# mat-lee/tetris-reinforcement-learning

Hardware: NVIDIA B200
Metric: placements/sec (movegen) (higher is better)
Workload: dtype u16

## Files before the change

### __graft_entry__.py

```python
import os
import sys

ROOT = os.path.dirname(os.path.abspath(__file__))
if ROOT not in sys.path:
    sys.path.insert(0, ROOT)


def build():
    from tetris_reinforcement_learning_b200 import build as b
    so = b.build(force=b.needs_build())
    from oracle import oracle
    oracle.build()
    import tetris_reinforcement_learning_b200
    from tetris_reinforcement_learning_b200 import _native
    _native.lib()
    print("built", so)


def smoke():
    import numpy as np
    import torch
    assert torch.cuda.is_available(), "smoke() needs a CUDA device"
    from oracle import oracle
    from tetris_reinforcement_learning_b200 import env, move_generation, synth
    from tetris_reinforcement_learning_b200.state import games_equal

    boards, cur, alt = synth.movegen_workload(64, seed=1, caves=True)
    dev = torch.device("cuda:0")
    d_mask = torch.empty((boards.shape[0], 362), dtype=torch.int32, device=dev)
    d_n = torch.empty(boards.shape[0], dtype=torch.int16, device=dev)
    move_generation.movegen_device(torch.from_numpy(boards.view(np.int16)).to(dev),
                                   torch.from_numpy(cur).to(dev), torch.from_numpy(alt).to(dev),
                                   d_mask, None, d_n, None)
    torch.cuda.synchronize()
    want_masks, want_n, _, total = oracle.movegen_batch(boards, cur, alt)
    assert np.array_equal(d_mask.cpu().numpy().view(np.uint32), want_masks), "movegen mask mismatch"
    assert np.array_equal(d_n.cpu().numpy().view(np.uint16), want_n)
    from tetris_reinforcement_learning_b200 import _native
    _native.lib().trl_movegen_warp_form(2)
    try:
        d_mask.zero_()
        move_generation.movegen_device(torch.from_numpy(boards.view(np.int16)).to(dev), torch.from_numpy(cur).to(dev),
                                       torch.from_numpy(alt).to(dev), d_mask, None, d_n, None)
        torch.cuda.synchronize()
    finally:
        _native.lib().trl_movegen_warp_form(-1)
    assert np.array_equal(d_mask.cpu().numpy().view(np.uint32), want_masks), "movegen mask mismatch (two-pass form)"
    assert np.array_equal(d_n.cpu().numpy().view(np.uint16), want_n)

    seed = 3
    games = env.game_setup_host(128, 0, seed)
    shadow = oracle.game_setup(128, 0, seed)
    for _ in range(8):
        pl = games["players"][np.arange(128), games["turn"]]
        res = move_generation.movegen_host(np.ascontiguousarray(pl["rows"]), pl["piece"].copy(),
                                           np.where(pl["held"] != 255, pl["held"], pl["queue"][:, 0]).astype(np.uint8),
                                           want_mask=False, want_moves=True, moves_cap=128)
        moves = res["moves"][:, 0].astype(np.uint16)
        env.env_step_host(games, moves, True, seed)
        oracle.env_step(shadow, moves, True, seed)
    assert games_equal(games, shadow).all(), "env step mismatch"

    from tetris_reinforcement_learning_b200 import architectures as arch, trunk
    from tetris_reinforcement_learning_b200.config import Config
    from tetris_reinforcement_learning_b200.selfplay import SelfPlayEngine
    torch.manual_seed(0)
    mc = arch.AlphaSameConfig(blocks=10, filters=16)
    net = arch.AlphaSame(mc).to(dev).eval()
    grids = (torch.rand((30, 1, 40, 10), device=dev) < 0.3).float()
    with torch.no_grad():
        ref = net.grid_features(grids)
    got = trunk.trunk_forward(trunk.pack_alphasame_trunk(net), grids.to(torch.bfloat16)).float()
    err = (got - ref).abs().max().item()
    assert err <= 0.03 * ref.abs().max().item() + 0.02, f"trunk mismatch {err}"
    cfg = Config(visual=False, ruleset="s2", model="pytorch", model_config=mc, MAX_ITER=8, training=True)
    eng = SelfPlayEngine(cfg, trunk.make_fused_evaluator(net), 64, device=dev, seed=1, feature_dtype=torch.bfloat16, max_rounds=4)
    eng.step(120)
    samples, ends = eng.drain()
    assert len(samples) > 0 and (eng.get_ctl()["status"] == 0).all(), "self-play step failed"
    from tetris_reinforcement_learning_b200 import trunk_wide
    wnet = arch.AuxBaseResNet(arch.AuxBaseResNetConfig(blocks=2, filters=32)).to(dev).eval()
    wt = trunk_wide.WideTrunk(trunk_wide.pack_wide_trunk(wnet), dev)
    with torch.no_grad():
        wref = wnet.opp_collapse(wnet._process_grid(grids)).flatten(1)
    wgot = trunk_wide.wide_trunk_forward(wt, grids.to(torch.bfloat16)).float()[:, 4 * 400:]
    wt.check()
    werr = (wgot - wref).abs().max().item()
    assert werr <= 0.04 * wref.abs().max().item() + 0.03, f"wide trunk mismatch {werr}"
    print(f"smoke ok: {boards.shape[0]} movegen calls ({total} placements) and 8 plies x 128 games bit-exact vs oracle; "
          f"trunk max err {err:.4f}, wide trunk max err {werr:.4f}; {len(samples)} searches, {len(ends)} games finished")


if __name__ == "__main__":
    build()
    if len(sys.argv) > 1 and sys.argv[1] == "smoke":
        smoke()
```

### tetris_reinforcement_learning_b200/csrc/movegen_warp.cu

```cuda
#include <cuda_runtime.h>
#include <stdint.h>

#include <mutex>

#include "trl_common.cuh"
#include "trl_tables.cuh"

namespace {

constexpr int kFifoCap = 768;
__constant__ int c_fifo_limit = kFifoCap;
constexpr int kCallsPerBlock = 8;
constexpr int kWarps = 2 * kCallsPerBlock;
constexpr int kVRows = TRL_MAP_H + 2;

struct PieceState {
    uint32_t vv[4][kVRows];
    uint32_t fu[4][kVRows];
    union {
        uint16_t fifo[kFifoCap];
        struct {
            uint32_t tsnap[4][32];
            uint32_t tp[4][2][36];
        };
// ... 333 lines not shown
        }
        const uint32_t b_nhi = e0w0[R] & 0xFFFFu, b_u = e0w0[R] >> 16, b_nlo = e0w1[R] & 0xFFFFu;
        const uint32_t b_any = b_nhi | b_u | b_nlo, b_win = b_u & ~b_nhi;
        all_n |= b_nhi | b_nlo; all_u |= b_u;
        const uint32_t l_n = late[R] & 0xFFFFu, l_u = late[R] >> 16, has_late = l_n | l_u;
        const uint32_t early_win = (q_any & q_win) | (~q_any & ((b_any & b_win) | (~b_any & i_win)));
        const uint32_t win = (early & early_win) | (~early & a_win);
        const uint32_t qn = (early & q_n) | (~early & a_n), qu = (early & q_u) | (~early & a_u);
        const uint32_t dec_u = (has_late & l_u & ~l_n & ~qn) | (~has_late & win);
        const uint32_t decided = (has_late & ((l_u & ~l_n & ~qn) | (l_n & ~l_u & ~qu))) | ~has_late;
        const uint32_t mixed = all_n & all_u & placed;
        const uint32_t suspect = seed_cell | (b_any & ~early);
        if (mixed & ~(decided & ~suspect)) undecided = true;
#ifdef TRL_MOVEGEN_STATS
        if (__any_sync(kAll, mixed & ~early)) TRL_REASON(11);
        if (__any_sync(kAll, mixed & suspect)) TRL_REASON(12);
        if (__any_sync(kAll, mixed & ~suspect & ~decided)) TRL_REASON(13);
#endif
        ulk[R] = ((all_u & ~mixed) | (dec_u & mixed)) & 0xFFFFu;
    }
    if (__any_sync(kAll, undecided)) { TRL_REASON(14); return false; }
    TRL_REASON(15);
    ulkA = ulk[0] | (ulk[2] << 16);
    ulkB = ulk[1] | (ulk[3] << 16);
    return true;
}

constexpr uint32_t kMinos[7][4] = {
    {TRL_PK(0, 0, 1, 0, 1, 1, 2, 1), TRL_PK(1, 1, 1, 2, 2, 0, 2, 1), TRL_PK(0, 1, 1, 1, 1, 2, 2, 2), TRL_PK(0, 1, 0, 2, 1, 0, 1, 1)},
    {TRL_PK(0, 1, 1, 1, 2, 0, 2, 1), TRL_PK(1, 0, 1, 1, 1, 2, 2, 2), TRL_PK(0, 1, 0, 2, 1, 1, 2, 1), TRL_PK(0, 0, 1, 0, 1, 1, 1, 2)},
    {TRL_PK(0, 0, 0, 1, 1, 0, 1, 1), TRL_PK(0, 0, 0, 1, 1, 0, 1, 1), TRL_PK(0, 0, 0, 1, 1, 0, 1, 1), TRL_PK(0, 0, 0, 1, 1, 0, 1, 1)},
    {TRL_PK(0, 1, 1, 0, 1, 1, 2, 0), TRL_PK(1, 0, 1, 1, 2, 1, 2, 2), TRL_PK(0, 2, 1, 1, 1, 2, 2, 1), TRL_PK(0, 0, 0, 1, 1, 1, 1, 2)},
    {TRL_PK(0, 1, 1, 1, 2, 1, 3, 1), TRL_PK(2, 0, 2, 1, 2, 2, 2, 3), TRL_PK(0, 2, 1, 2, 2, 2, 3, 2), TRL_PK(1, 0, 1, 1, 1, 2, 1, 3)},
    {TRL_PK(0, 0, 0, 1, 1, 1, 2, 1), TRL_PK(1, 0, 1, 1, 1, 2, 2, 0), TRL_PK(0, 1, 1, 1, 2, 1, 2, 2), TRL_PK(0, 2, 1, 0, 1, 1, 1, 2)},
    {TRL_PK(0, 1, 1, 0, 1, 1, 2, 1), TRL_PK(1, 0, 1, 1, 1, 2, 2, 1), TRL_PK(0, 1, 1, 1, 1, 2, 2, 1), TRL_PK(0, 1, 1, 0, 1, 1, 1, 2)},
};

template <int TYPE, int R>
__device__ __forceinline__ uint32_t validity_row(const uint32_t (&e)[4]) {
    constexpr uint32_t mm = kMinos[TYPE][R];
    constexpr int c0 = mm & 15, r0 = (mm >> 4) & 15, c1 = (mm >> 8) & 15, r1 = (mm >> 12) & 15;
    constexpr int c2 = (mm >> 16) & 15, r2 = (mm >> 20) & 15, c3 = (mm >> 24) & 15, r3 = (mm >> 28) & 15;
    return 0x3FFFu & (e[r0] >> c0) & (e[r1] >> c1) & (e[r2] >> c2) & (e[r3] >> c3);
}

template <int TYPE>
__device__ __forceinline__ void validity_rows(const uint32_t (&e)[4], uint32_t (&v)[4]) {
    v[0] = validity_row<TYPE, 0>(e);
    v[1] = validity_row<TYPE, 1>(e);
    v[2] = validity_row<TYPE, 2>(e);
    v[3] = validity_row<TYPE, 3>(e);
}

template <bool SPECIAL, class St>
__device__ __forceinline__ bool search_piece_rows(St& S, const uint16_t* rows, int hi, int type, bool via_hold, uint32_t* mask) {
    const int lane = threadIdx.x & 31;
    const int sx = trl_spawn_x(type);
    const bool is_T = (type == P_T);
    const int my = lane + kWin0;
    uint32_t e[4];
#pragma unroll
    for (int k = 0; k < 4; ++k) e[k] = trl_empty_row(rows, my - 2 + k) << 2;
    uint32_t VA = 0u, VB = 0u;
    if (SPECIAL && TRL_ROWS_SPECIAL_V) {
        uint32_t v[4];
        switch (type) {
            case 0: validity_rows<0>(e, v); break;
            case 1: validity_rows<1>(e, v); break;
            case 2: validity_rows<2>(e, v); break;
            case 3: validity_rows<3>(e, v); break;
            case 4: validity_rows<4>(e, v); break;
            case 5: validity_rows<5>(e, v); break;
            default: validity_rows<6>(e, v); break;
        }
        VA = v[0] | (v[2] << 16);
        VB = v[1] | (v[3] << 16);
    } else {
#pragma unroll 1
    for (int r = 0; r < 4; ++r) {
        const uint32_t m4 = c_minos[type][r];
        uint32_t acc = 0x3FFFu;
#pragma unroll
        for (int m = 0; m < 4; ++m) {
            const uint32_t co = (m4 >> (8 * m)) & 15u, ro = (m4 >> (8 * m + 4)) & 15u;
            const uint32_t ek = ro == 0 ? e[0] : (ro == 1 ? e[1] : (ro == 2 ? e[2] : e[3]));
            acc &= ek >> co;
        }
        const uint32_t sh = acc << (16 * (r >> 1));
        if (r & 1) VB |= sh; else VA |= sh;
    }
    }
    {
        const int pad = lane < 2 ? lane : lane + 32;
        S.vv[0][lane + 2] = VA << 2;
        S.vv[1][lane + 2] = VB << 2;
        if (lane < 4) { S.vv[0][pad] = 0u; S.vv[1][pad] = 0u; }
#pragma unroll
        for (int r = 0; r < 4; ++r) {
            S.fu[r][lane + 2] = 0u;
            if (lane < 4) S.fu[r][pad] = 0u;
        }
    }
    const uint32_t v_spawn = __shfl_sync(0xffffffffu, VA, TRL_SPAWN_Y + 2 - kWin0);
    if (via_hold && !((v_spawn >> (sx + 2)) & 1u)) return true;
    const int slane = max(hi - (int)c_matrix_size[type], TRL_SPAWN_Y) + 2 - kWin0;
    const uint32_t vs = __shfl_sync(0xffffffffu, VA, slane);
    if (!((vs >> (sx + 2)) & 1u)) return true;
// ... 91 lines not shown
                        __syncwarp();
                        const uint32_t d = S.fu[nrot][lane + 2];
                        const uint32_t k0 = (((nrot & 1) ? a0B : a0A) >> (16 * (nrot >> 1))) & 0xFFFFu;
                        if (round < 8) tt[((round * 4 + nrot) * 3 + kd) * 32 + lane] |= d | k0;
                        S.fu[nrot][lane + 2] = saved | d;
                        a0A |= sA; a0B |= sB;
                        __syncwarp();
                    }
                } trace_end{S, ttrace, nrot, kd, lane, tround, t_saved, t_a0A, t_a0B, a0A, a0B};
#endif
                const uint32_t Vn = ((nrot & 1) ? VB : VA) >> (16 * (nrot >> 1));
                const uint32_t c0 = ne & Vn;
                const uint32_t c0s = c0 << (16 * (nrot >> 1));
                if (nrot & 1) a0B |= c0s; else a0A |= c0s;
                uint32_t rem = ne & ~c0;
                if (!__any_sync(0xffffffffu, rem)) continue;
                const TrlKicks& K = c_kicks[tab][r][kd];
                const int kn = K.n;
                const uint32_t* vt = &S.vv[nrot & 1][lane + 2];
                const int vsh = 2 + 16 * (nrot >> 1);
                uint32_t* at = &S.fu[nrot][lane + 2];
#pragma unroll 1
                for (int ki = 1; ki < kn; ++ki) {
                    TRL_STAT(5);
                    const int kx = K.k[ki][0], ky = K.k[ki][1];
                    const uint32_t cand = rem & (vt[-ky] >> (kx + vsh));
                    rem &= ~cand;
                    if (cand) {
                        uint32_t arr = (cand << 4) >> (4 - kx);
                        if (is_T && kd != 1 && ki == kn - 1) arr <<= 16;
                        atomicOr(&at[-ky], arr);
                    }
                    if (!__any_sync(0xffffffffu, rem)) break;
                }
            }
        }
        }
#ifdef TRL_T_TRACE
        ++tround;
#endif
        __syncwarp();
        {
            const uint32_t f0 = S.fu[0][lane + 2], f1 = S.fu[1][lane + 2], f2 = S.fu[2][lane + 2], f3 = S.fu[3][lane + 2];
#ifdef TRL_MOVEGEN_STATS
            if (is_T && stat_2 == 1) {
                const uint32_t stA = VA & ~dA, stB = VB & ~dB;
                const uint32_t mA = (((f0 | a0A) & (f0 >> 16)) & 0xFFFFu) | ((((f2 << 16) | a0A) & f2) & 0xFFFF0000u);
                const uint32_t mB = (((f1 | a0B) & (f1 >> 16)) & 0xFFFFu) | ((((f3 << 16) | a0B) & f3) & 0xFFFF0000u);
                if (__any_sync(0xffffffffu, (mA & stA) | (mB & stB))) stat_6 = 1;
            }
#endif
            RA |= a0A | ((f0 | (f0 >> 16)) & 0xFFFFu) | ((f2 | (f2 >> 16)) << 16);
            RB |= a0B | ((f1 | (f1 >> 16)) & 0xFFFFu) | ((f3 | (f3 >> 16)) << 16);
            if (is_T && ++kick_rounds == 2) {
                S.tsnap[0][lane] = f0 | (a0A & 0xFFFFu); S.tsnap[1][lane] = f1 | (a0B & 0xFFFFu);
                S.tsnap[2][lane] = f2 | (a0A >> 16); S.tsnap[3][lane] = f3 | (a0B >> 16);
                S.fu[0][lane + 2] = 0u; S.fu[1][lane + 2] = 0u; S.fu[2][lane + 2] = 0u; S.fu[3][lane + 2] = 0u;
                a0A = 0u; a0B = 0u;
                snapped = true;
                __syncwarp();
            }
        }
    }
#ifdef TRL_MOVEGEN_STATS
    if (lane == 0) {
        atomicAdd(&g_fast_stats[2], (unsigned long long)stat_2); atomicAdd(&g_fast_stats[3], (unsigned long long)stat_3);
        atomicAdd(&g_fast_stats[4], (unsigned long long)stat_4); atomicAdd(&g_fast_stats[5], (unsigned long long)stat_5);
        atomicAdd(&g_fast_stats[6], (unsigned long long)stat_6);
    }
#endif
    if (__any_sync(0xffffffffu, lane < 2 && (RA | RB))) return false;
    const uint32_t placedA = RA & ~dA, placedB = RB & ~dB;
#ifdef TRL_T_TRACE
    if (ttrace) {
        ttrace[8 * 4 * 3 * 32 + 0 * 32 + lane] = placedA & 0xFFFFu; ttrace[8 * 4 * 3 * 32 + 1 * 32 + lane] = placedB & 0xFFFFu;
        ttrace[8 * 4 * 3 * 32 + 2 * 32 + lane] = placedA >> 16; ttrace[8 * 4 * 3 * 32 + 3 * 32 + lane] = placedB >> 16;
        ttrace[8 * 4 * 3 * 32 + 4 * 32 + lane] = (uint32_t)rows[lane] | (lane < TRL_ROWS - 32 ? (uint32_t)rows[lane + 32] << 16 : 0u);
    }
#endif
    uint32_t flagA = 0u, flagB = 0u, ulkA = 0u, ulkB = 0u;
    if (is_T) {
        uint32_t nA = a0A, nB = a0B, uA = 0u, uB = 0u;
#pragma unroll
        for (int r = 0; r < 4; ++r) {
            const uint32_t fw = S.fu[r][lane + 2] | (snapped ? S.tsnap[r][lane] : 0u);
            const uint32_t n = (fw & 0xFFFFu) << (16 * (r >> 1)), u = (fw >> 16) << (16 * (r >> 1));
            if (r & 1) { nB |= n; uB |= u; } else { nA |= n; uA |= u; }
        }
        flagA = nA | uA; flagB = nB | uB;
        ulkA = uA; ulkB = uB;
        const uint32_t mxA = nA & uA & placedA, mxB = nB & uB & placedB;
        const uint32_t mixed_rots = (__any_sync(0xffffffffu, mxA & 0xFFFFu) ? 1u : 0u) | (__any_sync(0xffffffffu, mxB & 0xFFFFu) ? 2u : 0u) |
                                    (__any_sync(0xffffffffu, mxA >> 16) ? 4u : 0u) | (__any_sync(0xffffffffu, mxB >> 16) ? 8u : 0u);
        if (mixed_rots) {
            if (!t_order_decide(S, lane, VA, VB, slane, sx + 2, placedA, placedB, a0A, a0B, snapped, mixed_rots, ulkA, ulkB)) return false;
        }
    }
    const int pbase = c_plane_base[type];
    const int nrot_planes = c_plane_nrot[type];
    const bool zsi = (type == P_Z || type == P_S || type == P_I);
    if (my < TRL_MAP_H - 1) {
        const int n_rot = (type == P_O) ? 1 : 4;
#pragma unroll 1
        for (int rot = 0; rot < n_rot; ++rot) {
            const uint32_t placed = (((rot & 1) ? placedB : placedA) >> (16 * (rot >> 1))) & 0xFFFFu;
            if (!placed) continue;
            int row = my - 2;
            uint32_t bits = placed;
            if (zsi) {
                if (rot == 2) row += 1;
                else if (rot == 3) bits >>= 1;
            }
            if (!is_T) {
                or_chunk(mask, pbase + rot % nrot_planes, row, bits & 0x7FFu);
            } else {
                const uint32_t f = (((rot & 1) ? flagB : flagA) >> (16 * (rot >> 1))) & placed;
                const uint32_t u = (((rot & 1) ? ulkB : ulkA) >> (16 * (rot >> 1))) & 0xFFFFu;
                or_chunk(mask, pbase + rot, row, (placed & ~f) & 0x7FFu);
                or_chunk(mask, pbase + 4 + rot, row, (f & ~u) & 0x7FFu);
                or_chunk(mask, pbase + 8 + rot, row, (f & u) & 0x7FFu);
            }
        }
    }
    return true;
}

__device__ __noinline__ bool search_piece_rows_call(PieceState& S, const uint16_t* rows, int type, bool via_hold, uint32_t* mask) {
    return search_piece_rows<false>(S, rows, first_block_row(rows, threadIdx.x & 31), type, via_hold, mask);
}

__device__ __noinline__ void search_piece_fifo(PieceState& S, const uint16_t* rows, int type, bool via_hold, uint32_t* mask,
                                  uint32_t& status, const uint32_t (*kpack)[4][3][2]) {
    const int lane = threadIdx.x & 31;
    uint32_t minos[4];
#pragma unroll
    for (int r = 0; r < 4; ++r) minos[r] = c_minos[type][r];
    const int sx = trl_spawn_x(type);
    if (via_hold && !trl_fits(rows, minos[0], sx, TRL_SPAWN_Y)) return;

#pragma unroll
    for (int r = 0; r < 4; ++r) {
        for (int my = lane; my < kVRows; my += 32) {
            S.vv[r][my] = (my < TRL_MAP_H) ? trl_valid_row(rows, minos[r], my) : 0u;
            S.fu[r][my] = 0u;
        }
    }
    int hi = TRL_ROWS;
    for (int i = lane; i < TRL_ROWS; i += 32)
        if (rows[i] & TRL_FULL_ROW) hi = min(hi, i);
    hi = __reduce_min_sync(0xffffffffu, hi);
    const int sy = max(hi - (int)c_matrix_size[type], TRL_SPAWN_Y);
    __syncwarp();
    if (!((S.vv[0][sy + 2] >> (sx + 2)) & 1u)) return;

    const bool is_T = (type == P_T);
    const bool rotates = (type != P_O);
    const int tab = (type == P_I) ? 1 : 0;

    uint32_t head = 0, tail = 1;
    if (lane == 0) S.fifo[0] = (uint16_t)fifo_pack(sx + 2, sy + 2, 0, 0, 0);
    __syncwarp();

    while (head != tail) {
        const int n = min(32u, tail - head);
        const uint32_t e = (lane < n) ? S.fifo[(head + lane) % kFifoCap] : 0u;
        const int mx = e & 15, my = (e >> 4) & 63, rot = (e >> 10) & 3;
        const uint32_t bit = 1u << mx;
        const uint32_t w = S.vv[rot][my];
        const bool stuck = !(S.vv[rot][my + 1] & bit);
        const bool need = (lane < n) && !((w >> 16) & bit) && (w & bit);
        const uint32_t m_need = __ballot_sync(0xffffffffu, need);
        const int first = m_need ? (__ffs(m_need) - 1) : 32;
        if (is_T) {
            const bool emit = (lane < n) && (lane <= first) && ((e >> 12) & 1u) && stuck;
            const uint32_t m_emit = __ballot_sync(0xffffffffu, emit);
            if (m_emit) {
                const bool u = (e >> 13) & 1u;
                const uint32_t m_true = __ballot_sync(0xffffffffu, emit && u);
                if (m_true == 0u || m_true == m_emit) {
                    if (emit) flag_cell(&S.fu[rot][my], bit, u);
                } else if (emit) {
                    const uint32_t grp = __match_any_sync(m_emit, e & 0xFFFu);
                    if ((31 - __clz(grp)) == lane) flag_cell(&S.fu[rot][my], bit, u);
                    else atomicOr(&S.fu[rot][my], bit);
                }
// ... 180 lines not shown
                        if (mixed && lane != l) { __syncwarp(); continue; }
                        uint32_t iv = Im[0] | Im[1] | Im[2];
                        while (iv) {
                            const int ex = __ffs(iv) - 1;
                            iv &= iv - 1;
#pragma unroll
                            for (int kd = 0; kd < 3; ++kd) {
                                if (!((Im[kd] >> ex) & 1u)) continue;
                                const int ki = ((k0[kd] >> ex) & 1u) | (((k1[kd] >> ex) & 1u) << 1) | (((k2[kd] >> ex) & 1u) << 2);
                                const int kn = c_kicks[tab][frot][kd].n;
                                const bool nulk = (kd != 1 && ki == kn - 1);
                                const int kx = (int)(((*kpack)[frot][kd][0] >> (4 * ki)) & 15u) - 2;
                                const int ky = (int)(((*kpack)[frot][kd][1] >> (4 * ki)) & 15u) - 2;
                                flag_cell(&S.fu[(frot + kd + 1) & 3][ky_row - ky], 1u << (ex + kx), nulk);
                            }
                        }
                        __syncwarp();
                    }
                }
            }
            __syncwarp();
        }
    }
    __syncwarp();

    const int pbase = c_plane_base[type];
    const int nrot_planes = c_plane_nrot[type];
    const bool zsi = (type == P_Z || type == P_S || type == P_I);
    for (int rot = 0; rot < 4; ++rot) {
        if (type == P_O && rot > 0) break;
        for (int my = 2 + lane; my < TRL_MAP_H - 1; my += 32) {
            const uint32_t wv = S.vv[rot][my];
            const uint32_t placed = (wv >> 16) & ~S.vv[rot][my + 1] & 0xFFFFu;
            if (!placed) continue;
            int row = my - 2;
            uint32_t bits = placed;
            if (zsi) {
                if (rot == 2) row += 1;
                else if (rot == 3) bits >>= 1;
            }
            if (!is_T) {
                or_chunk(mask, pbase + rot % nrot_planes, row, bits & 0x7FFu);
            } else {
                const uint32_t fw = S.fu[rot][my];
                const uint32_t f = fw & placed, u = fw >> 16;
                or_chunk(mask, pbase + rot, row, (placed & ~f) & 0x7FFu);
                or_chunk(mask, pbase + 4 + rot, row, (f & ~u) & 0x7FFu);
                or_chunk(mask, pbase + 8 + rot, row, (f & u) & 0x7FFu);
            }
        }
    }
}

__device__ __forceinline__ void search_piece_warp(PieceState& S, const uint16_t* rows, int type, bool via_hold, uint32_t* mask,
                                                  uint32_t& status, const uint32_t (*kpack)[4][3][2], bool exact_only = false) {
    if (!exact_only && c_fast_path && c_fifo_limit == kFifoCap) {
        const bool done = search_piece_rows_call(S, rows, type, via_hold, mask);
        if ((threadIdx.x & 31) == 0) atomicAdd(&g_fast_stats[done ? 0 : 1], 1ull);
        if (done) return;
        __syncwarp();
    }
    search_piece_fifo(S, rows, type, via_hold, mask, status, kpack);
}

__device__ __noinline__ void write_move_list(const CallState& C, int lane, uint16_t* mv, int cap) {
    uint32_t nz = 0u;
#pragma unroll
    for (int j = 0; j < 12; ++j) {
        const int w = lane + 32 * j;
        if (w < TRL_MASK_WORDS && C.mask[w]) nz |= 1u << j;
    }
    while (nz) {
        const int j = __ffs(nz) - 1;
        nz &= nz - 1;
        const int w = lane + 32 * j;
        uint32_t m = C.mask[w];
        int pos = (int)C.lbase[(w * 683) >> 13] + (int)C.woff[w];
        while (m) {
            const int b = __ffs(m) - 1;
            m &= m - 1;
            if (pos < cap) mv[pos] = (uint16_t)(w * 32 + b);
            ++pos;
        }
    }
}

template <int MODE = 0>
__device__ __forceinline__ void write_call_outputs(CallState& C, int i, int lane, uint32_t* __restrict__ mask_bits,
                                                   uint16_t* __restrict__ moves, int moves_cap,
                                                   uint16_t* __restrict__ n_moves, uint32_t* __restrict__ status,
                                                   uint16_t* __restrict__ compact, unsigned long long compact_cap,
                                                   unsigned long long* __restrict__ compact_total,
                                                   unsigned long long* __restrict__ offsets) {
    if (C.skip) {
        if (lane == 0) {
            if (n_moves) n_moves[i] = 0;
            if (status) status[i] = 0;
            if (compact) offsets[i] = 0;
        }
        return;
    }
    const int w0 = lane * 12;
    const bool want_list = MODE == 0 ? (compact != nullptr || moves != nullptr) : (MODE == 2);
    int cnt = 0;
    uint32_t* gm = mask_bits ? mask_bits + (size_t)i * TRL_MASK_WORDS : nullptr;
#pragma unroll 1
// ... 148 lines not shown
    __shared__ uint32_t s_kpack[2][4][3][2];
    const int tid = threadIdx.x, warp = tid >> 5, lane = tid & 31;
    SoloState& S = reinterpret_cast<SoloState*>(smem_raw)[warp];
    CallState& C = S.C;
    if (tid < 24) {
        const int t = tid / 12, r = (tid / 3) % 4, kd = tid % 3;
        const TrlKicks& K = c_kicks[t][r][kd];
        uint32_t px = 0, py = 0;
        for (int ki = 0; ki < K.n; ++ki) {
            px |= (uint32_t)(K.k[ki][0] + 2) << (4 * ki);
            py |= (uint32_t)(K.k[ki][1] + 2) << (4 * ki);
        }
        s_kpack[t][r][kd][0] = px;
        s_kpack[t][r][kd][1] = py;
    }
    __syncthreads();
    const int n_items = call_list ? (int)call_count[0] : n;
#pragma unroll 1
    for (int j = blockIdx.x * kSoloWarps + warp; j < n_items; j += gridDim.x * kSoloWarps) {
        const int i = call_list ? call_list[j] : j;
        int c, a, skip;
        zero_mask(C, lane);
        stage_call(C, i, lane, boards, cur, alt, games, index, c, a, skip);
        __syncwarp();
        if (!skip) {
            uint32_t st = 0;
#pragma unroll 1
            for (int which = 0; which < 2; ++which) {
                const int type = which ? a : c;
                if (type == TRL_NONE || (which && a == c)) continue;
                search_piece_warp(S.P, C.rows, type, which != 0, C.mask, st, &s_kpack[type == P_I ? 1 : 0],
                                  call_list != nullptr && type == P_T);
                __syncwarp();
            }
            st = __reduce_or_sync(0xffffffffu, st);
            if (st && lane == 0) C.status |= st;
            __syncwarp();
        }
        write_call_outputs(C, i, lane, mask_bits, moves, moves_cap, n_moves, status, compact, compact_cap, compact_total, offsets);
        __syncwarp();
    }
}

#ifndef TRL_ROWS_SPECIAL
#define TRL_ROWS_SPECIAL 1
#endif
#ifndef TRL_ROWS_WARPS
#define TRL_ROWS_WARPS 4
#endif
#ifndef TRL_ROWS_MIN_BLOCKS
#define TRL_ROWS_MIN_BLOCKS 10
#endif
constexpr int kRowsWarps = TRL_ROWS_WARPS;

struct RowsState {
    uint32_t vv[2][kWinRows];
    uint32_t fu[4][kWinRows];
    uint32_t tsnap[4][32];
    uint32_t tp[4][2][36];
};

struct RowsWarp {
    RowsState P;
    CallState C;
};

template <bool WANT_LIST>
__global__ void __launch_bounds__(kRowsWarps * 32, TRL_ROWS_MIN_BLOCKS)
movegen_rows_kernel(const uint16_t* __restrict__ boards, const uint8_t* __restrict__ cur,
                    const uint8_t* __restrict__ alt, const TrlGame* __restrict__ games,
                    const int32_t* __restrict__ index, int n, uint32_t* __restrict__ mask_bits,
                    uint16_t* __restrict__ moves, int moves_cap, uint16_t* __restrict__ n_moves,
                    uint32_t* __restrict__ status, uint16_t* __restrict__ compact, unsigned long long compact_cap,
                    unsigned long long* __restrict__ compact_total, unsigned long long* __restrict__ offsets,
                    int32_t* __restrict__ undecided, uint32_t* __restrict__ undecided_count) {
    extern __shared__ __align__(16) uint8_t smem_raw[];
    const int tid = threadIdx.x, warp = tid >> 5, lane = tid & 31;
    RowsWarp& S = reinterpret_cast<RowsWarp*>(smem_raw)[warp];
    CallState& C = S.C;
    const int i = blockIdx.x * kRowsWarps + warp;
    if (i >= n) return;
    int c, a, skip;
    zero_mask(C, lane);
    stage_call(C, i, lane, boards, cur, alt, games, index, c, a, skip);
    __syncwarp();
    if (!skip) {
        const int hi = first_block_row(C.rows, lane);
        bool ok = true;
#pragma unroll 1
        for (int which = 0; which < 2 && ok; ++which) {
            const int type = which ? a : c;
            if (type == TRL_NONE || (which && a == c)) continue;
            ok = search_piece_rows<TRL_ROWS_SPECIAL != 0>(S.P, C.rows, hi, type, which != 0, C.mask);
            if (ok) TRL_REASON(0); else TRL_REASON(1);
            __syncwarp();
        }
        if (!ok) {
            if (lane == 0) undecided[atomicAdd(undecided_count, 1u)] = i;
            return;
        }
    }
    write_call_outputs<WANT_LIST ? 2 : 1>(C, i, lane, mask_bits, moves, moves_cap, n_moves, status, compact, compact_cap, compact_total, offsets);
}

constexpr int kListSlots = 16;

__device__ __forceinline__ void slot_barrier(int slot) {
    asm volatile("bar.sync %0, 64;" ::"r"(slot) : "memory");
}

__global__ void __launch_bounds__(kListSlots * 64)
movegen_list_kernel(const TrlGame* __restrict__ games, const int32_t* __restrict__ index,
                    const int32_t* __restrict__ list, uint32_t* __restrict__ count_done,
                    uint16_t* __restrict__ moves, int moves_cap, uint16_t* __restrict__ n_moves, int rounds,
                    TrlSearchCtl* __restrict__ ctl) {
    extern __shared__ __align__(16) uint8_t smem_raw[];
    PieceState* ps = reinterpret_cast<PieceState*>(smem_raw);
    CallState* cs = reinterpret_cast<CallState*>(smem_raw + sizeof(PieceState) * kListSlots * 2);
    __shared__ int s_ticket[kListSlots];
    __shared__ uint32_t s_kpack[2][4][3][2];
    const int tid = threadIdx.x, warp = tid >> 5, lane = tid & 31;
    const int slot = warp >> 1, which = warp & 1;
    __shared__ int s_count;
    __shared__ unsigned s_warps_done;
    if (tid == 32) { s_count = (int)count_done[0]; s_warps_done = 0u; }
    {
        if (tid < 24) {
            const int t = tid / 12, r = (tid / 3) % 4, kd = tid % 3;
            const TrlKicks& K = c_kicks[t][r][kd];
            uint32_t px = 0, py = 0;
            for (int ki = 0; ki < K.n; ++ki) {
                px |= (uint32_t)(K.k[ki][0] + 2) << (4 * ki);
                py |= (uint32_t)(K.k[ki][1] + 2) << (4 * ki);
            }
            s_kpack[t][r][kd][0] = px;
            s_kpack[t][r][kd][1] = py;
        }
    }
    __syncthreads();
    const int count = s_count;
    const int n_work = min((int)gridDim.x, (count + kListSlots * rounds - 1) / (kListSlots * rounds));
    if ((int)blockIdx.x < n_work) {
        CallState& C = cs[slot];
        while (true) {
            if (which == 0 && lane == 0) s_ticket[slot] = (int)atomicAdd(&count_done[2], 1u);
            slot_barrier(slot);
            const int j = s_ticket[slot];
            if (j >= count) break;
            const int g = list[j];
            const int gi = index[g];
            for (int w2 = which * 32 + lane; w2 < TRL_MASK_WORDS + 2; w2 += 64) C.mask[w2] = 0u;
            if (which == 0) {
                const TrlPlayer& p = games[gi].players[games[gi].turn & 1];
                for (int r = lane; r < TRL_ROWS; r += 32) C.rows[r] = p.rows[r];
                int c = p.piece;
// ... 79 lines not shown
    if (!rc) rc = trl_check(cudaMemcpyToSymbol(g_fast_stats, z, sizeof(z)));
    answered[0] = h[0]; answered[1] = h[1];
#ifdef TRL_MOVEGEN_STATS
    for (int k = 2; k < 16; ++k) answered[k] = h[k];
#endif
    return rc;
}

extern "C" int trl_debug_movegen_t_trace(uint32_t* device_buffer, unsigned cap) {
#ifdef TRL_T_TRACE
    unsigned zero = 0;
    int rc = trl_check(cudaMemcpyToSymbol(g_t_trace, &device_buffer, sizeof(device_buffer)));
    if (!rc) rc = trl_check(cudaMemcpyToSymbol(g_t_trace_cap, &cap, sizeof(cap)));
    if (!rc) rc = trl_check(cudaMemcpyToSymbol(g_t_trace_n, &zero, sizeof(zero)));
    return rc ? rc : kTTraceWords;
#else
    (void)device_buffer; (void)cap;
    return TRL_E_ARG;
#endif
}

extern "C" int trl_debug_movegen_fifo_limit(int limit) {
    if (limit < 1 || limit > kFifoCap) limit = kFifoCap;
    g_fifo_limit_host = limit;
    return trl_check(cudaMemcpyToSymbol(c_fifo_limit, &limit, sizeof(int)));
}

int trl_launch_movegen_listed(const TrlGame* games, const int32_t* index, const int32_t* list, uint32_t* count_done,
                              uint16_t* moves, int moves_cap, uint16_t* n_moves, TrlSearchCtl* ctl, cudaStream_t stream) {
    if (!games || !index || !list || !count_done || !moves || !n_moves || moves_cap <= 0) return TRL_E_ARG;
    const size_t smem = sizeof(PieceState) * kListSlots * 2 + sizeof(CallState) * kListSlots;
    static int n_sm = 0;
    if (!n_sm) {
        int dev = 0, sms = 0;
        int rc = trl_check(cudaGetDevice(&dev));
        if (!rc) rc = trl_check(cudaDeviceGetAttribute(&sms, cudaDevAttrMultiProcessorCount, dev));
        if (!rc) rc = trl_check(cudaFuncSetAttribute(movegen_list_kernel, cudaFuncAttributeMaxDynamicSharedMemorySize, (int)smem));
        if (rc) return rc;
        n_sm = sms;
    }
    movegen_list_kernel<<<n_sm, kListSlots * 64, smem, stream>>>(games, index, list, count_done, moves, moves_cap, n_moves,
                                                                g_list_rounds, ctl);
    return trl_check(cudaGetLastError());
}

static int g_form = -1;
extern "C" void trl_movegen_warp_form(int form) { g_form = form; }

struct TwoPassScratch { cudaStream_t stream; uint32_t* buf; size_t cap; bool used; };
static TwoPassScratch g_scratch[8];

static std::mutex g_scratch_mutex;

static uint32_t* two_pass_scratch(cudaStream_t stream, int n) {
    std::lock_guard<std::mutex> lock(g_scratch_mutex);
    TwoPassScratch* slot = nullptr;
    for (auto& e : g_scratch) if (e.used && e.stream == stream) { slot = &e; break; }
    if (!slot) for (auto& e : g_scratch) if (!e.used) { slot = &e; e.used = true; e.stream = stream; e.buf = nullptr; e.cap = 0; break; }
    if (!slot) return nullptr;
    const size_t need = (size_t)n + 16;
    if (slot->cap < need) {
        cudaStreamCaptureStatus cs = cudaStreamCaptureStatusNone;
        if (cudaStreamIsCapturing(stream, &cs) != cudaSuccess || cs != cudaStreamCaptureStatusNone) return nullptr;
        if (slot->buf) { cudaStreamSynchronize(stream); cudaFree(slot->buf); slot->buf = nullptr; slot->cap = 0; }
        if (cudaMalloc(&slot->buf, need * sizeof(uint32_t)) != cudaSuccess) { cudaGetLastError(); return nullptr; }
        slot->cap = need;
    }
    return slot->buf;
}

int trl_launch_movegen_warp(const uint16_t* boards, const uint8_t* cur, const uint8_t* alt, const TrlGame* games,
                            const int32_t* index, int n, uint32_t* mask_bits, uint16_t* moves, int moves_cap,
                            uint16_t* n_moves, uint32_t* status, cudaStream_t stream, uint16_t* compact,
                            unsigned long long compact_cap, unsigned long long* compact_total,
                            unsigned long long* offsets) {
    static int n_sm = 0;
    static bool configured = false;
    const size_t smem_warp = sizeof(PieceState) * kWarps + sizeof(CallState) * kCallsPerBlock;
    const size_t smem_solo = sizeof(SoloState) * kSoloWarps;
    const size_t smem_rows = sizeof(RowsWarp) * kRowsWarps;
    if (!configured) {
        int dev = 0;
        int rc = trl_check(cudaGetDevice(&dev));
        if (!rc) rc = trl_check(cudaDeviceGetAttribute(&n_sm, cudaDevAttrMultiProcessorCount, dev));
        if (!rc) rc = trl_check(cudaFuncSetAttribute(movegen_warp_kernel, cudaFuncAttributeMaxDynamicSharedMemorySize, (int)smem_warp));
        if (!rc) rc = trl_check(cudaFuncSetAttribute(movegen_solo_kernel, cudaFuncAttributeMaxDynamicSharedMemorySize, (int)smem_solo));
        if (!rc) rc = trl_check(cudaFuncSetAttribute(movegen_solo_kernel, cudaFuncAttributePreferredSharedMemoryCarveout, 100));
        if (!rc) rc = trl_check(cudaFuncSetAttribute(movegen_rows_kernel<false>, cudaFuncAttributeMaxDynamicSharedMemorySize, (int)smem_rows));
        if (!rc) rc = trl_check(cudaFuncSetAttribute(movegen_rows_kernel<false>, cudaFuncAttributePreferredSharedMemoryCarveout, 100));
        if (!rc) rc = trl_check(cudaFuncSetAttribute(movegen_rows_kernel<true>, cudaFuncAttributeMaxDynamicSharedMemorySize, (int)smem_rows));
        if (!rc) rc = trl_check(cudaFuncSetAttribute(movegen_rows_kernel<true>, cudaFuncAttributePreferredSharedMemoryCarveout, 100));
        if (rc) return rc;
        configured = true;
    }
    int form = g_form < 0 ? (n >= 3 * 4736 ? 2 : 0) : g_form;
    if (form == 2 && (!g_fast_path_host || g_fifo_limit_host != kFifoCap)) form = 1;
    uint32_t* scratch = form == 2 ? two_pass_scratch(stream, n) : nullptr;
    if (form == 2 && !scratch) form = 1;
    if (form == 2) {
        int rc = trl_check(cudaMemsetAsync(scratch, 0, sizeof(uint32_t), stream));
        if (rc) return rc;
        if (moves || compact)
            movegen_rows_kernel<true><<<(n + kRowsWarps - 1) / kRowsWarps, kRowsWarps * 32, smem_rows, stream>>>(
                boards, cur, alt, games, index, n, mask_bits, moves, moves_cap, n_moves, status, compact, compact_cap,
                compact_total, offsets, (int32_t*)(scratch + 16), scratch);
        else
            movegen_rows_kernel<false><<<(n + kRowsWarps - 1) / kRowsWarps, kRowsWarps * 32, smem_rows, stream>>>(
                boards, cur, alt, games, index, n, mask_bits, moves, moves_cap, n_moves, status, compact, compact_cap,
                compact_total, offsets, (int32_t*)(scratch + 16), scratch);
        rc = trl_check(cudaGetLastError());
        if (rc) return rc;
        const int blocks = min(8 * n_sm, (n + kSoloWarps - 1) / kSoloWarps);
        movegen_solo_kernel<<<blocks, kSoloWarps * 32, smem_solo, stream>>>(
            boards, cur, alt, games, index, n, mask_bits, moves, moves_cap, n_moves, status, compact, compact_cap,
            compact_total, offsets, (const int32_t*)(scratch + 16), scratch);
        return trl_check(cudaGetLastError());
    }
    if (form == 1) {
        const int blocks = (n + kSoloWarps - 1) / kSoloWarps;
        movegen_solo_kernel<<<blocks, kSoloWarps * 32, smem_solo, stream>>>(boards, cur, alt, games, index, n, mask_bits, moves,
                                                                           moves_cap, n_moves, status, compact, compact_cap,
                                                                           compact_total, offsets, nullptr, nullptr);
        int rc = trl_check(cudaGetLastError());
        return rc;
    }
    const int blocks = (n + kCallsPerBlock - 1) / kCallsPerBlock;
    movegen_warp_kernel<<<blocks, kWarps * 32, smem_warp, stream>>>(boards, cur, alt, games, index, n, mask_bits, moves,
                                                                   moves_cap, n_moves, status, compact, compact_cap,
                                                                   compact_total, offsets, nullptr, nullptr);
    return trl_check(cudaGetLastError());
}
```

Baseline: 10.50 billion.

## Split T-piece order resolution into deferred passes instead of full fallback

The rows kernel no longer runs T-spin order resolution inline. Calls whose only failure is the T piece get their partial mask saved and are deferred to a new persistent T-order kernel, and calls it still cannot decide go to an exact FIFO kernel. Only other failures fall back to the legacy solo kernel. The aim is to shrink the rows kernel's shared-memory footprint (tsnap/tp removed) and to stop sending T-heavy calls down the expensive full re-search. In exchange it adds two extra launches, atomic work queues, and partial-mask storage traffic.

```diff
diff --git a/__graft_entry__.py b/__graft_entry__.py
--- a/__graft_entry__.py
+++ b/__graft_entry__.py
@@ -45,7 +45,7 @@
         torch.cuda.synchronize()
     finally:
         _native.lib().trl_movegen_warp_form(-1)
-    assert np.array_equal(d_mask.cpu().numpy().view(np.uint32), want_masks), "movegen mask mismatch (two-pass form)"
+    assert np.array_equal(d_mask.cpu().numpy().view(np.uint32), want_masks), "movegen mask mismatch (pass form)"
     assert np.array_equal(d_n.cpu().numpy().view(np.uint16), want_n)
 
     seed = 3
diff --git a/tetris_reinforcement_learning_b200/csrc/movegen_warp.cu b/tetris_reinforcement_learning_b200/csrc/movegen_warp.cu
--- a/tetris_reinforcement_learning_b200/csrc/movegen_warp.cu
+++ b/tetris_reinforcement_learning_b200/csrc/movegen_warp.cu
@@ -409,7 +409,7 @@
     v[3] = validity_row<TYPE, 3>(e);
 }
 
-template <bool SPECIAL, class St>
+template <bool SPECIAL, bool T_ORDER, class St>
 __device__ __forceinline__ bool search_piece_rows(St& S, const uint16_t* rows, int hi, int type, bool via_hold, uint32_t* mask) {
     const int lane = threadIdx.x & 31;
     const int sx = trl_spawn_x(type);
@@ -607,13 +607,15 @@
 #endif
             RA |= a0A | ((f0 | (f0 >> 16)) & 0xFFFFu) | ((f2 | (f2 >> 16)) << 16);
             RB |= a0B | ((f1 | (f1 >> 16)) & 0xFFFFu) | ((f3 | (f3 >> 16)) << 16);
-            if (is_T && ++kick_rounds == 2) {
-                S.tsnap[0][lane] = f0 | (a0A & 0xFFFFu); S.tsnap[1][lane] = f1 | (a0B & 0xFFFFu);
-                S.tsnap[2][lane] = f2 | (a0A >> 16); S.tsnap[3][lane] = f3 | (a0B >> 16);
-                S.fu[0][lane + 2] = 0u; S.fu[1][lane + 2] = 0u; S.fu[2][lane + 2] = 0u; S.fu[3][lane + 2] = 0u;
-                a0A = 0u; a0B = 0u;
-                snapped = true;
-                __syncwarp();
+            if constexpr (T_ORDER) {
+                if (is_T && ++kick_rounds == 2) {
+                    S.tsnap[0][lane] = f0 | (a0A & 0xFFFFu); S.tsnap[1][lane] = f1 | (a0B & 0xFFFFu);
+                    S.tsnap[2][lane] = f2 | (a0A >> 16); S.tsnap[3][lane] = f3 | (a0B >> 16);
+                    S.fu[0][lane + 2] = 0u; S.fu[1][lane + 2] = 0u; S.fu[2][lane + 2] = 0u; S.fu[3][lane + 2] = 0u;
+                    a0A = 0u; a0B = 0u;
+                    snapped = true;
+                    __syncwarp();
+                }
             }
         }
     }
@@ -638,7 +640,8 @@
         uint32_t nA = a0A, nB = a0B, uA = 0u, uB = 0u;
 #pragma unroll
         for (int r = 0; r < 4; ++r) {
-            const uint32_t fw = S.fu[r][lane + 2] | (snapped ? S.tsnap[r][lane] : 0u);
+            uint32_t fw = S.fu[r][lane + 2];
+            if constexpr (T_ORDER) fw |= snapped ? S.tsnap[r][lane] : 0u;
             const uint32_t n = (fw & 0xFFFFu) << (16 * (r >> 1)), u = (fw >> 16) << (16 * (r >> 1));
             if (r & 1) { nB |= n; uB |= u; } else { nA |= n; uA |= u; }
         }
@@ -648,7 +651,8 @@
         const uint32_t mixed_rots = (__any_sync(0xffffffffu, mxA & 0xFFFFu) ? 1u : 0u) | (__any_sync(0xffffffffu, mxB & 0xFFFFu) ? 2u : 0u) |
                                     (__any_sync(0xffffffffu, mxA >> 16) ? 4u : 0u) | (__any_sync(0xffffffffu, mxB >> 16) ? 8u : 0u);
         if (mixed_rots) {
-            if (!t_order_decide(S, lane, VA, VB, slane, sx + 2, placedA, placedB, a0A, a0B, snapped, mixed_rots, ulkA, ulkB)) return false;
+            if constexpr (!T_ORDER) return false;
+            else if (!t_order_decide(S, lane, VA, VB, slane, sx + 2, placedA, placedB, a0A, a0B, snapped, mixed_rots, ulkA, ulkB)) return false;
         }
     }
     const int pbase = c_plane_base[type];
@@ -681,11 +685,11 @@
 }
 
 __device__ __noinline__ bool search_piece_rows_call(PieceState& S, const uint16_t* rows, int type, bool via_hold, uint32_t* mask) {
-    return search_piece_rows<false>(S, rows, first_block_row(rows, threadIdx.x & 31), type, via_hold, mask);
-}
-
-__device__ __noinline__ void search_piece_fifo(PieceState& S, const uint16_t* rows, int type, bool via_hold, uint32_t* mask,
-                                  uint32_t& status, const uint32_t (*kpack)[4][3][2]) {
+    return search_piece_rows<false, true>(S, rows, first_block_row(rows, threadIdx.x & 31), type, via_hold, mask);
+}
+
+__device__ __forceinline__ void search_piece_fifo_body(PieceState& S, const uint16_t* rows, int type, bool via_hold, uint32_t* mask,
+                                                       uint32_t& status, const uint32_t (*kpack)[4][3][2]) {
     const int lane = threadIdx.x & 31;
     uint32_t minos[4];
 #pragma unroll
@@ -972,6 +976,11 @@
     }
 }
 
+__device__ __noinline__ void search_piece_fifo(PieceState& S, const uint16_t* rows, int type, bool via_hold, uint32_t* mask,
+                                              uint32_t& status, const uint32_t (*kpack)[4][3][2]) {
+    search_piece_fifo_body(S, rows, type, via_hold, mask, status, kpack);
+}
+
 __device__ __forceinline__ void search_piece_warp(PieceState& S, const uint16_t* rows, int type, bool via_hold, uint32_t* mask,
                                                   uint32_t& status, const uint32_t (*kpack)[4][3][2], bool exact_only = false) {
     if (!exact_only && c_fast_path && c_fifo_limit == kFifoCap) {
@@ -1226,18 +1235,47 @@
 #define TRL_ROWS_MIN_BLOCKS 10
 #endif
 constexpr int kRowsWarps = TRL_ROWS_WARPS;
+constexpr int kTWarps = 4;
+
+enum : int { kCntLegacy = 0, kCntDeferred = 1, kCntExact = 2, kTicketOrder = 3, kTicketExact = 4, kCounters = 16 };
+struct PassLists {
+    uint32_t* counts;
+    int32_t* legacy;
+    int32_t* deferred;
+    int32_t* exact;
+    uint32_t* partial;
+    unsigned deferred_cap;
+};
 
 struct RowsState {
     uint32_t vv[2][kWinRows];
     uint32_t fu[4][kWinRows];
-    uint32_t tsnap[4][32];
-    uint32_t tp[4][2][36];
 };
 
 struct RowsWarp {
     RowsState P;
     CallState C;
 };
+
+__device__ __forceinline__ void store_mask(const CallState& C, uint32_t* __restrict__ g, int lane) {
+#pragma unroll 1
+    for (int w = lane; w < TRL_MASK_WORDS; w += 32) g[w] = C.mask[w];
+}
+
+__device__ __forceinline__ void load_mask(CallState& C, const uint32_t* __restrict__ g, int lane) {
+#pragma unroll 1
+    for (int w = lane; w < TRL_MASK_WORDS + 2; w += 32) C.mask[w] = w < TRL_MASK_WORDS ? g[w] : 0u;
+}
+
+__device__ __forceinline__ uint32_t* partial_mask(const PassLists& pl, uint32_t* mask_bits, int i, unsigned j) {
+    return pl.partial ? pl.partial + (size_t)j * TRL_MASK_WORDS : mask_bits + (size_t)i * TRL_MASK_WORDS;
+}
+
+__device__ __forceinline__ unsigned next_item(uint32_t* ticket, int lane) {
+    unsigned j = 0;
+    if (lane == 0) j = atomicAdd(ticket, 1u);
+    return __shfl_sync(0xffffffffu, j, 0);
+}
 
 template <bool WANT_LIST>
 __global__ void __launch_bounds__(kRowsWarps * 32, TRL_ROWS_MIN_BLOCKS)
@@ -1247,7 +1285,7 @@
                     uint16_t* __restrict__ moves, int moves_cap, uint16_t* __restrict__ n_moves,
                     uint32_t* __restrict__ status, uint16_t* __restrict__ compact, unsigned long long compact_cap,
                     unsigned long long* __restrict__ compact_total, unsigned long long* __restrict__ offsets,
-                    int32_t* __restrict__ undecided, uint32_t* __restrict__ undecided_count) {
+                    const PassLists pl) {
     extern __shared__ __align__(16) uint8_t smem_raw[];
     const int tid = threadIdx.x, warp = tid >> 5, lane = tid & 31;
     RowsWarp& S = reinterpret_cast<RowsWarp*>(smem_raw)[warp];
@@ -1260,21 +1298,126 @@
     __syncwarp();
     if (!skip) {
         const int hi = first_block_row(C.rows, lane);
-        bool ok = true;
+        bool legacy = false, t_deferred = false;
 #pragma unroll 1
-        for (int which = 0; which < 2 && ok; ++which) {
+        for (int which = 0; which < 2 && !legacy; ++which) {
             const int type = which ? a : c;
             if (type == TRL_NONE || (which && a == c)) continue;
-            ok = search_piece_rows<TRL_ROWS_SPECIAL != 0>(S.P, C.rows, hi, type, which != 0, C.mask);
+            const bool ok = search_piece_rows<TRL_ROWS_SPECIAL != 0, false>(S.P, C.rows, hi, type, which != 0, C.mask);
             if (ok) TRL_REASON(0); else TRL_REASON(1);
             __syncwarp();
-        }
+            if (!ok) {
+                if (type == P_T) t_deferred = true;
+                else legacy = true;
+            }
+        }
+        if (t_deferred && !legacy) {
+            unsigned j = 0;
+            if (lane == 0) j = atomicAdd(&pl.counts[kCntDeferred], 1u);
+            j = __shfl_sync(0xffffffffu, j, 0);
+            if (j < pl.deferred_cap) {
+                store_mask(C, partial_mask(pl, mask_bits, i, j), lane);
+                if (lane == 0) pl.deferred[j] = i;
+                return;
+            }
+            legacy = true;
+        }
+        if (legacy) {
+            if (lane == 0) pl.legacy[atomicAdd(&pl.counts[kCntLegacy], 1u)] = i;
+            return;
+        }
+    }
+    write_call_outputs<WANT_LIST ? 2 : 1>(C, i, lane, mask_bits, moves, moves_cap, n_moves, status, compact, compact_cap, compact_total, offsets);
+}
+
+__device__ __forceinline__ void stage_wall_kpack(uint32_t (&kp)[4][3][2], int tid) {
+    if (tid < 12) {
+        const int r = tid / 3, kd = tid % 3;
+        const TrlKicks& K = c_kicks[0][r][kd];
+        uint32_t px = 0, py = 0;
+        for (int ki = 0; ki < K.n; ++ki) {
+            px |= (uint32_t)(K.k[ki][0] + 2) << (4 * ki);
+            py |= (uint32_t)(K.k[ki][1] + 2) << (4 * ki);
+        }
+        kp[r][kd][0] = px;
+        kp[r][kd][1] = py;
+    }
+}
+
+__device__ __forceinline__ bool stage_deferred(CallState& C, const PassLists& pl, unsigned j, int lane, const uint16_t* __restrict__ boards,
+                                               const uint8_t* __restrict__ cur, const uint8_t* __restrict__ alt,
+                                               const TrlGame* __restrict__ games, const int32_t* __restrict__ index,
+                                               uint32_t* mask_bits, int& i) {
+    i = pl.deferred[j];
+    int c, a, skip;
+    stage_call(C, i, lane, boards, cur, alt, games, index, c, a, skip);
+    load_mask(C, partial_mask(pl, mask_bits, i, j), lane);
+    __syncwarp();
+    return c != P_T;
+}
+
+template <bool WANT_LIST>
+__global__ void __launch_bounds__(kTWarps * 32, 8)
+movegen_t_order_kernel(const uint16_t* __restrict__ boards, const uint8_t* __restrict__ cur,
+                       const uint8_t* __restrict__ alt, const TrlGame* __restrict__ games,
+                       const int32_t* __restrict__ index, uint32_t* __restrict__ mask_bits,
+                       uint16_t* __restrict__ moves, int moves_cap, uint16_t* __restrict__ n_moves,
+                       uint32_t* __restrict__ status, uint16_t* __restrict__ compact, unsigned long long compact_cap,
+                       unsigned long long* __restrict__ compact_total, unsigned long long* __restrict__ offsets,
+                       const PassLists pl) {
+    extern __shared__ __align__(16) uint8_t smem_raw[];
+    const int tid = threadIdx.x, warp = tid >> 5, lane = tid & 31;
+    SoloState& S = reinterpret_cast<SoloState*>(smem_raw)[warp];
+    CallState& C = S.C;
+    const unsigned count = min(pl.counts[kCntDeferred], pl.deferred_cap);
+#pragma unroll 1
+    while (true) {
+        const unsigned j = next_item(&pl.counts[kTicketOrder], lane);
+        if (j >= count) break;
+        int i;
+        const bool via_hold = stage_deferred(C, pl, j, lane, boards, cur, alt, games, index, mask_bits, i);
+        const bool ok = search_piece_rows<true, true>(S.P, C.rows, first_block_row(C.rows, lane), P_T, via_hold, C.mask);
+        __syncwarp();
         if (!ok) {
-            if (lane == 0) undecided[atomicAdd(undecided_count, 1u)] = i;
-            return;
-        }
-    }
-    write_call_outputs<WANT_LIST ? 2 : 1>(C, i, lane, mask_bits, moves, moves_cap, n_moves, status, compact, compact_cap, compact_total, offsets);
+            if (lane == 0) pl.exact[atomicAdd(&pl.counts[kCntExact], 1u)] = (int32_t)j;
+            continue;
+        }
+        write_call_outputs<WANT_LIST ? 2 : 1>(C, i, lane, mask_bits, moves, moves_cap, n_moves, status, compact, compact_cap, compact_total, offsets);
+        __syncwarp();
+    }
+}
+
+template <bool WANT_LIST>
+__global__ void __launch_bounds__(kTWarps * 32, 8)
+movegen_t_exact_kernel(const uint16_t* __restrict__ boards, const uint8_t* __restrict__ cur,
+                       const uint8_t* __restrict__ alt, const TrlGame* __restrict__ games,
+                       const int32_t* __restrict__ index, uint32_t* __restrict__ mask_bits,
+                       uint16_t* __restrict__ moves, int moves_cap, uint16_t* __restrict__ n_moves,
+                       uint32_t* __restrict__ status, uint16_t* __restrict__ compact, unsigned long long compact_cap,
+                       unsigned long long* __restrict__ compact_total, unsigned long long* __restrict__ offsets,
+                       const PassLists pl) {
+    extern __shared__ __align__(16) uint8_t smem_raw[];
+    __shared__ uint32_t s_kpack[4][3][2];
+    const int tid = threadIdx.x, warp = tid >> 5, lane = tid & 31;
+    SoloState& S = reinterpret_cast<SoloState*>(smem_raw)[warp];
+    CallState& C = S.C;
+    stage_wall_kpack(s_kpack, tid);
+    __syncthreads();
+    const unsigned count = pl.counts[kCntExact];
+#pragma unroll 1
+    while (true) {
+        const unsigned e = next_item(&pl.counts[kTicketExact], lane);
+        if (e >= count) break;
+        int i;
+        const bool via_hold = stage_deferred(C, pl, (unsigned)pl.exact[e], lane, boards, cur, alt, games, index, mask_bits, i);
+        uint32_t st = 0;
+        search_piece_fifo_body(S.P, C.rows, P_T, via_hold, C.mask, st, &s_kpack);
+        st = __reduce_or_sync(0xffffffffu, st);
+        if (st && lane == 0) C.status |= st;
+        __syncwarp();
+        write_call_outputs<WANT_LIST ? 2 : 1>(C, i, lane, mask_bits, moves, moves_cap, n_moves, status, compact, compact_cap, compact_total, offsets);
+        __syncwarp();
+    }
 }
 
 constexpr int kListSlots = 16;
@@ -1460,13 +1603,12 @@
 
 static std::mutex g_scratch_mutex;
 
-static uint32_t* two_pass_scratch(cudaStream_t stream, int n) {
+static uint32_t* two_pass_scratch(cudaStream_t stream, size_t need) {
     std::lock_guard<std::mutex> lock(g_scratch_mutex);
     TwoPassScratch* slot = nullptr;
     for (auto& e : g_scratch) if (e.used && e.stream == stream) { slot = &e; break; }
     if (!slot) for (auto& e : g_scratch) if (!e.used) { slot = &e; e.used = true; e.stream = stream; e.buf = nullptr; e.cap = 0; break; }
     if (!slot) return nullptr;
-    const size_t need = (size_t)n + 16;
     if (slot->cap < need) {
         cudaStreamCaptureStatus cs = cudaStreamCaptureStatusNone;
         if (cudaStreamIsCapturing(stream, &cs) != cudaSuccess || cs != cudaStreamCaptureStatusNone) return nullptr;
@@ -1477,16 +1619,38 @@
     return slot->buf;
 }
 
+static unsigned g_partial_cap_debug = 0;
+extern "C" int trl_debug_movegen_partial_cap(int cap) {
+    g_partial_cap_debug = cap > 0 ? (unsigned)cap : 0u;
+    return 0;
+}
+
+static uint32_t* g_last_counts = nullptr;
+static unsigned g_last_deferred_cap = 0;
+
+extern "C" int trl_debug_movegen_pass_counts(uint32_t* counts) {
+    if (!counts || !g_last_counts) return TRL_E_ARG;
+    uint32_t h[kCounters];
+    int rc = trl_check(cudaDeviceSynchronize());
+    if (!rc) rc = trl_check(cudaMemcpy(h, g_last_counts, sizeof(h), cudaMemcpyDeviceToHost));
+    if (rc) return rc;
+    counts[0] = h[kCntDeferred] < g_last_deferred_cap ? h[kCntDeferred] : g_last_deferred_cap;
+    counts[1] = h[kCntExact];
+    counts[2] = h[kCntLegacy];
+    return 0;
+}
+
 int trl_launch_movegen_warp(const uint16_t* boards, const uint8_t* cur, const uint8_t* alt, const TrlGame* games,
                             const int32_t* index, int n, uint32_t* mask_bits, uint16_t* moves, int moves_cap,
                             uint16_t* n_moves, uint32_t* status, cudaStream_t stream, uint16_t* compact,
                             unsigned long long compact_cap, unsigned long long* compact_total,
                             unsigned long long* offsets) {
-    static int n_sm = 0;
+    static int n_sm = 0, t_order_blocks = 0, t_exact_blocks = 0;
     static bool configured = false;
     const size_t smem_warp = sizeof(PieceState) * kWarps + sizeof(CallState) * kCallsPerBlock;
     const size_t smem_solo = sizeof(SoloState) * kSoloWarps;
     const size_t smem_rows = sizeof(RowsWarp) * kRowsWarps;
+    const size_t smem_t = sizeof(SoloState) * kTWarps;
     if (!configured) {
         int dev = 0;
         int rc = trl_check(cudaGetDevice(&dev));
@@ -1498,30 +1662,52 @@
         if (!rc) rc = trl_check(cudaFuncSetAttribute(movegen_rows_kernel<false>, cudaFuncAttributePreferredSharedMemoryCarveout, 100));
         if (!rc) rc = trl_check(cudaFuncSetAttribute(movegen_rows_kernel<true>, cudaFuncAttributeMaxDynamicSharedMemorySize, (int)smem_rows));
         if (!rc) rc = trl_check(cudaFuncSetAttribute(movegen_rows_kernel<true>, cudaFuncAttributePreferredSharedMemoryCarveout, 100));
+        for (const void* f : {(const void*)movegen_t_order_kernel<false>, (const void*)movegen_t_order_kernel<true>,
+                              (const void*)movegen_t_exact_kernel<false>, (const void*)movegen_t_exact_kernel<true>}) {
+            if (!rc) rc = trl_check(cudaFuncSetAttribute(f, cudaFuncAttributeMaxDynamicSharedMemorySize, (int)smem_t));
+            if (!rc) rc = trl_check(cudaFuncSetAttribute(f, cudaFuncAttributePreferredSharedMemoryCarveout, 100));
+        }
+        if (!rc) rc = trl_check(cudaOccupancyMaxActiveBlocksPerMultiprocessor(&t_order_blocks, movegen_t_order_kernel<false>, kTWarps * 32, smem_t));
+        if (!rc) rc = trl_check(cudaOccupancyMaxActiveBlocksPerMultiprocessor(&t_exact_blocks, movegen_t_exact_kernel<false>, kTWarps * 32, smem_t));
         if (rc) return rc;
         configured = true;
     }
     int form = g_form < 0 ? (n >= 3 * 4736 ? 2 : 0) : g_form;
     if (form == 2 && (!g_fast_path_host || g_fifo_limit_host != kFifoCap)) form = 1;
-    uint32_t* scratch = form == 2 ? two_pass_scratch(stream, n) : nullptr;
+    unsigned deferred_cap = (unsigned)n;
+    if (!mask_bits) deferred_cap = (unsigned)min(n, max(64 * 1024, n / 8));
+    if (g_partial_cap_debug) deferred_cap = min(deferred_cap, g_partial_cap_debug);
+    const size_t lists = kCounters + 3 * (size_t)n;
+    uint32_t* scratch = form == 2 ? two_pass_scratch(stream, lists + (mask_bits ? 0 : (size_t)deferred_cap * TRL_MASK_WORDS)) : nullptr;
     if (form == 2 && !scratch) form = 1;
     if (form == 2) {
-        int rc = trl_check(cudaMemsetAsync(scratch, 0, sizeof(uint32_t), stream));
+        const PassLists pl{scratch, (int32_t*)scratch + kCounters, (int32_t*)scratch + kCounters + n,
+                           (int32_t*)scratch + kCounters + 2 * (size_t)n, mask_bits ? nullptr : scratch + lists, deferred_cap};
+        g_last_counts = scratch;
+        g_last_deferred_cap = deferred_cap;
+        int rc = trl_check(cudaMemsetAsync(scratch, 0, kCounters * sizeof(uint32_t), stream));
         if (rc) return rc;
-        if (moves || compact)
-            movegen_rows_kernel<true><<<(n + kRowsWarps - 1) / kRowsWarps, kRowsWarps * 32, smem_rows, stream>>>(
-                boards, cur, alt, games, index, n, mask_bits, moves, moves_cap, n_moves, status, compact, compact_cap,
-                compact_total, offsets, (int32_t*)(scratch + 16), scratch);
-        else
-            movegen_rows_kernel<false><<<(n + kRowsWarps - 1) / kRowsWarps, kRowsWarps * 32, smem_rows, stream>>>(
-                boards, cur, alt, games, index, n, mask_bits, moves, moves_cap, n_moves, status, compact, compact_cap,
-                compact_total, offsets, (int32_t*)(scratch + 16), scratch);
+        const bool want_list = moves || compact;
+        const int rows_blocks = (n + kRowsWarps - 1) / kRowsWarps;
+        (want_list ? movegen_rows_kernel<true> : movegen_rows_kernel<false>)<<<rows_blocks, kRowsWarps * 32, smem_rows, stream>>>(
+            boards, cur, alt, games, index, n, mask_bits, moves, moves_cap, n_moves, status, compact, compact_cap,
+            compact_total, offsets, pl);
+        rc = trl_check(cudaGetLastError());
+        if (rc) return rc;
+        (want_list ? movegen_t_order_kernel<true> : movegen_t_order_kernel<false>)<<<t_order_blocks * n_sm, kTWarps * 32, smem_t, stream>>>(
+            boards, cur, alt, games, index, mask_bits, moves, moves_cap, n_moves, status, compact, compact_cap,
+            compact_total, offsets, pl);
+        rc = trl_check(cudaGetLastError());
+        if (rc) return rc;
+        (want_list ? movegen_t_exact_kernel<true> : movegen_t_exact_kernel<false>)<<<t_exact_blocks * n_sm, kTWarps * 32, smem_t, stream>>>(
+            boards, cur, alt, games, index, mask_bits, moves, moves_cap, n_moves, status, compact, compact_cap,
+            compact_total, offsets, pl);
         rc = trl_check(cudaGetLastError());
         if (rc) return rc;
         const int blocks = min(8 * n_sm, (n + kSoloWarps - 1) / kSoloWarps);
         movegen_solo_kernel<<<blocks, kSoloWarps * 32, smem_solo, stream>>>(
             boards, cur, alt, games, index, n, mask_bits, moves, moves_cap, n_moves, status, compact, compact_cap,
-            compact_total, offsets, (const int32_t*)(scratch + 16), scratch);
+            compact_total, offsets, pl.legacy, pl.counts + kCntLegacy);
         return trl_check(cudaGetLastError());
     }
     if (form == 1) {
```

New measurement: 11.15 billion, median of 6. +6.2%, better.
